# gillesdegottex/percivaltts

Hardware: AMD Instinct MI355X
Metric: acoustic frames/sec per WGAN-GP critic+gen step (higher is better)
Workload: dtype f32

## Files before the change

include/percival_hip.h:

```cpp
#ifndef PERCIVAL_HIP_H
#define PERCIVAL_HIP_H

#include <stddef.h>
#include <stdint.h>

#ifdef __cplusplus
extern "C" {
#endif

#define PTTS_OK            0
#define PTTS_EINVAL       -1
#define PTTS_ELAUNCH      -2
#define PTTS_EWORKSPACE   -3
#define PTTS_EDEVICE      -4

#define PTTS_IN_NONE     0
#define PTTS_IN_LRELU    1
#define PTTS_IN_MASKMUL  2

#define PTTS_PAD_SAME    0
#define PTTS_PAD_CAUSAL  1

#define PTTS_ACT_NONE    0
#define PTTS_ACT_LRELU   1
// ... 126 lines not shown
                                     int Kin, int N, int M, long long lda, long long ldb, int in_mode, float alpha,
                                     void* stream);
int ptts_dense_wgrad_reduce_grouped(const ptts_dense_wgrad_reduce_desc* descs, int n, void* stream);
int ptts_dense_wgrad_bf16x6(const float* A, const float* dY, const float* mask_src, const float* in_scale,
                            const float* in_shift, float* C, float* colsum_b, void* workspace, size_t workspace_bytes,
                            int Kin, int N, int M, long long lda, long long ldb, long long ldc, int in_mode, float alpha,
                            void* stream);
int ptts_dense_bf16x6(const float* A, const void* planes, const float* bias, float* C, int M, int N, int K,
                      long long lda, long long ldc, int in_mode, const float* in_scale, const float* in_shift,
                      const float* mask_src, float alpha, int accumulate, const float* out_mask, void* stream);
int ptts_dense_bf16x6_res(const float* A, const void* planes, const float* bias, float* C, int M, int N, int K,
                          long long lda, long long ldc, int in_mode, const float* in_scale, const float* in_shift,
                          const float* mask_src, float alpha, const float* res, int res_rows, long long ldr,
                          const float* out_mask, void* stream);
int ptts_dense_bf16x6_stats_rows(int M, int N);
int ptts_dense_bf16x6_stats(const float* A, const void* planes, const float* bias, float* C, int M, int N, int K,
                            long long lda, long long ldc, int in_mode, const float* in_scale, const float* in_shift,
                            float alpha, double* stats, int capacity_rows, int* nrows_out, void* stream);
int ptts_dense_bf16x6_bwd_affine(const float* A, const void* planes, float* C, int M, int N, int K, long long lda, long long ldc,
                                 const float* z, const float* scale, const float* shift, float alpha,
                                 double* stats, int capacity_rows, int* nrows_out, void* stream);
int ptts_partial_rows_sum(const double* partials, int nrows, int ncols, double* out, void* stream);
int ptts_dft_mirror(float* Ap, int NB, int B, int Cin, int Kh, void* stream);

int ptts_conv1d_freq_kernel_planes(const float* w, const float* tw, void* planes, int NB, int KW, int Cin, int N, int Kh, void* stream);

int ptts_transpose_batched(const float* src, float* dst, int nb, int rows, int cols, void* stream);
int ptts_conv1d_freq_wgrad_combine(const float* out2, float* dW, int KW, int Cin, int N, int Kh, void* stream);

size_t ptts_conv1d_freq_wgrad_inverse_workspace_bytes(int KW, int Cin, int N);
int ptts_conv1d_freq_wgrad_inverse(const float* Gt, const float* t2, float* dW, void* workspace, size_t workspace_bytes,
                                   int NB, int NBp, int KW, int Cin, int N, int Kh, void* stream);

int ptts_dense_bf16x6_batched(const float* A, long long strideA, const void* planes, long long stride_planes_bytes,
                              const float* bias, float* C, long long strideC, int nbatch, int M, int N, int K,
                              long long lda, long long ldc, int planes_count, void* stream);
int ptts_set_dense_batched_resident(int on);
int ptts_dense_batched_resident_eligible(long long strideA, int M, int N, int K, int planes_count);
int ptts_dense_tn_bf16x6_batched(const float* A, long long strideA, const float* B, long long strideB, float* C, long long strideC,
                                 int nbatch, int M, int Kin, int N, long long lda, long long ldb, long long ldc, int planes_count,
                                 void* stream);

int ptts_split3_frames(const float* x, void* p1, void* p2, void* p3, int B, int T, int C, int pad_left, int pad_right,
                       int Cp, void* stream);
int ptts_split3_weight_t(const float* w, void* p1, void* p2, void* p3, int KW, int C, int N, int Cp, void* stream);
int ptts_conv1d_bf16x6(const void* a1, const void* a2, const void* a3, const void* bt1, const void* bt2, const void* bt3,
                       const float* bias, float* y, int B, int T, int KW, int Cp, int N, void* stream);

int ptts_split3_frames_t(const float* x, void* p1, void* p2, void* p3, int B, int T, int C, int pad_left, int Tp, int Crows,
                         long long Pp, void* stream);
int ptts_conv1d_wgrad_bf16x6(const void* xt1, const void* xt2, const void* xt3, const void* yt1, const void* yt2,
                             const void* yt3, float* dw, int B, int T, int KW, int C, int N, int Crows, long long Pp,
                             void* stream);

int ptts_transpose_frames(const float* x, float* out, int B, int T, int C, int pad_left, int Tp, int Crows, long long Pp,
                          void* stream);
int ptts_conv1d_wgrad_t(const float* xt, const float* yt, float* dw, float* db, int B, int T, int KW, int C, int N, int Crows,
                        long long Pp, void* stream);

size_t ptts_colstats_workspace_bytes(long long rows, int C);
int ptts_colstats(const float* x, long long rows, int C,
                  int in_mode, const float* in_scale, const float* in_shift, const float* mask_src, float alpha,
                  double* sums , void* workspace, size_t workspace_bytes, void* stream);

int ptts_bn_finalize(const double* sums, long long count, const float* gamma, const float* beta,
                     float* moving_mean, float* moving_var, float eps, float momentum,
                     int training, int update_moving, int unbiased_moving, int C,
                     float* scale, float* shift, float* mean , float* rstd , void* stream);

int ptts_bn_batch_stats_supported(long long rows, int C);
// ... 168 lines not shown
```

percivaltts_amd/_hip.py:

```python
import ctypes
import os
import re

import torch

_HERE = os.path.dirname(os.path.abspath(__file__))
LIB_PATH = os.environ.get('PTTS_LIB_PATH') or os.path.join(_HERE, 'lib', 'libpercival_hip.so')
HEADER_PATH = os.environ.get('PTTS_HEADER_PATH') or os.path.join(_HERE, '..', 'include', 'percival_hip.h')


class HipLibraryError(RuntimeError):
    pass


_SCALARS = {'int': ctypes.c_int, 'unsigned': ctypes.c_uint, 'float': ctypes.c_float, 'double': ctypes.c_double,
            'size_t': ctypes.c_size_t, 'long long': ctypes.c_longlong, 'unsigned long long': ctypes.c_ulonglong}
_DECLARATOR = re.compile(r'(.*[\s*])(\w+)\s*(\[\s*\])?', re.S)


def _ctype(spelling, where):
    t = ' '.join(w for w in spelling.replace('*', ' * ').split() if w != 'const')
    if t.endswith('*'):
        return ctypes.c_char_p if t == 'char *' else ctypes.c_void_p
    if t not in _SCALARS:
# ... 23 lines not shown
                raise HipLibraryError('percival_hip.h: cannot read {!r}'.format(' '.join(line.split())))
            fields.extend((n.strip(), ctype) for n in [name] + more)
        return ''

    text = re.sub(r'typedef\s+struct\s+(\w+)\s*\{(.*?)\}\s*\1\s*;', struct, text, flags=re.S)
    for decl in filter(str.strip, text.split(';')):
        m = re.fullmatch(r'\s*(.+?)\b(ptts_\w+)\s*\((.*)\)\s*', decl, flags=re.S)
        if m is None:
            raise HipLibraryError('percival_hip.h: cannot read {!r}'.format(' '.join(decl.split())))
        args = [] if m.group(3).strip() == 'void' else [_declaration(a, decl)[1] for a in m.group(3).split(',')]
        functions[m.group(2)] = (_ctype(m.group(1), decl), args)
    return structs, functions


def read_header(path):
    if not os.path.exists(path):
        raise HipLibraryError('percival_hip.h not found at {}: it lies in include/ beside the package (or set PTTS_HEADER_PATH). '
                              'The binding is read from it.'.format(path))
    with open(path) as f:
        return parse_header(f.read())


_STRUCTS, SIGNATURES = read_header(HEADER_PATH)


def _structure(name, cname):
    return type(name, (ctypes.Structure,), {'_fields_': _STRUCTS[cname], '__doc__': 'struct {} of include/percival_hip.h.'.format(cname)})


WGradDesc = _structure('WGradDesc', 'ptts_wgrad_desc')
DenseWgradReduceDesc = _structure('DenseWgradReduceDesc', 'ptts_dense_wgrad_reduce_desc')
DenseSplitDesc = _structure('DenseSplitDesc', 'ptts_dense_split_desc')
Conv2dReduceDesc = _structure('Conv2dReduceDesc', 'ptts_conv2d_reduce_desc')

_lib = None


def lib():
    global _lib
    if _lib is None:
        if not os.path.exists(LIB_PATH):
            raise HipLibraryError(
                'libpercival_hip.so not found at {}: run `python -c "import __graft_entry__ as g; g.build()"` '
                '(or `make -C percivaltts_amd/csrc`). There is no CPU fallback.'.format(LIB_PATH))
        l = ctypes.CDLL(LIB_PATH)
        for name, (res, args) in SIGNATURES.items():
            fn = getattr(l, name)
            fn.restype = res
            fn.argtypes = args
        if os.environ.get('PTTS_DETERMINISTIC', '0') == '1':
            l.ptts_set_deterministic(1)
        _lib = l
    return _lib


def last_error():
    return lib().ptts_last_error().decode('utf8', 'replace')


class KernelTimer(object):
    active = None

    def __init__(self):
        self.records = []

    def __enter__(self):
# ... 72 lines not shown
```

percivaltts_amd/csrc/dense.hip:

```cpp
#include "common.h"
#include <cstdlib>

namespace ptts {
namespace dns {

typedef __bf16 bf16x8 __attribute__((ext_vector_type(8)));
typedef __bf16 bf16x4 __attribute__((ext_vector_type(4)));
typedef __bf16 bf16x2 __attribute__((ext_vector_type(2)));
typedef float f32x4 __attribute__((ext_vector_type(4)));
typedef float f32x2 __attribute__((ext_vector_type(2)));
typedef unsigned u32x2 __attribute__((ext_vector_type(2)));
typedef unsigned short u16;

constexpr int THREADS = 512;
constexpr int NBLK = 256;
constexpr int BK = 32;

#define DNS_PRODUCTS(X) X(2, 0) X(1, 1) X(0, 2) X(1, 0) X(0, 1) X(0, 0)
#define DNS_PRODUCTS_NPL(NPL, X) do { if (NPL == 3) { X(2, 0) X(1, 1) X(0, 2) X(1, 0) X(0, 1) } X(0, 0) } while (0)

__device__ __forceinline__ unsigned pk_bf16(float a, float b) {
    return __builtin_bit_cast(unsigned, __builtin_convertvector((f32x2){a, b}, bf16x2));
}
__device__ __forceinline__ void split3_pair(float a, float b, unsigned& p1, unsigned& p2, unsigned& p3) {
// ... 509 lines not shown
                for (int e = 0; e < 4; ++e) { row[n + e] = (double)ssum[e]; row[g.N + n + e] = (double)ssq[e]; }
            }
        }
    }
}

template <int MODE, bool AFFINE, int MT, int NPL>
static void dense_launch_kernel(bool xt, dim3 grid, hipStream_t st, const DenseArgs& g) {
    if constexpr (MT < 8) {
        if (xt) { hipLaunchKernelGGL((dense_bf16x6_kernel<MODE, AFFINE, MT, NPL, true>), grid, dim3(THREADS), 0, st, g); return; }
    }
    hipLaunchKernelGGL((dense_bf16x6_kernel<MODE, AFFINE, MT, NPL>), grid, dim3(THREADS), 0, st, g);
}

static int pick_mt(int M, int col_blocks) {
    static int forced = -1;
    if (forced < 0) { const char* e = getenv("PTTS_DENSE_MT"); forced = e ? atoi(e) : 0; }
    if (forced >= 4 && forced <= 8) return forced;
    int best = 8; double best_eff = -1.0;
    for (int mt = 4; mt <= 8; ++mt) {
        const long long blocks = (long long)((M + 16 * mt - 1) / (16 * mt)) * col_blocks;
        const long long rounds = (blocks + 255) / 256;
        const double eff = (double)M * col_blocks / (double)(rounds * 256 * 16 * mt);
        if (eff > best_eff + 1e-9) { best_eff = eff; best = mt; }
    }
    return best;
}

constexpr int RES_M = 128, RES_K = 128;
constexpr int RES_KS = RES_K / BK;
constexpr int RES_PL = RES_M * BK;
template <int NPL> constexpr size_t resident_lds_bytes() { return (size_t)RES_KS * NPL * RES_PL * sizeof(u16); }

template <int NPL, int MT = RES_M / 16, int KSC = 0>
__global__ __launch_bounds__(THREADS) void dense_bf16x6_resident_kernel(DenseArgs g, int slices, int items) {
    extern __shared__ __attribute__((aligned(16))) u16 lds_r[];
    const int tid = threadIdx.x, lane = tid & 63;
    const int wave = __builtin_amdgcn_readfirstlane(tid >> 6);
    const int li = lane & 15, lg = lane >> 4;
    const int KS = KSC ? KSC : g.KS;
    const size_t ps = (size_t)g.NT * KS * 512;
    const int stride = 8 * (int)gridDim.x;
    int item = 8 * (int)blockIdx.x + wave;
    const bool live = item < items;

    constexpr int NQ = RES_M * (RES_K / 4) / THREADS;
    f32x4 va[NQ];
#pragma unroll
    for (int j = 0; j < NQ; ++j) {
        const int q = tid + j * THREADS, row = q >> 5, k4 = 4 * (q & 31);
        const bool ok = row < g.M && k4 < g.K;
        va[j] = *reinterpret_cast<const f32x4*>(g.A + (ok ? (long long)row * g.lda + k4 : 0));
    }

    bf16x8 wf[RES_KS][2][NPL];
    auto load_w = [&](int it, int s) {
        const int z = it / slices, sl = it - z * slices;
        const u16* wp = g.planes + (long long)z * g.bsP + (((size_t)(2 * sl) * KS + s) * 64 + lane) * 8;
#pragma unroll
        for (int j = 0; j < 2; ++j)
#pragma unroll
            for (int p = 0; p < NPL; ++p) wf[s][j][p] = *reinterpret_cast<const bf16x8*>(wp + p * ps + (size_t)j * KS * 512);
    };
#pragma unroll
    for (int s = 0; s < RES_KS; ++s) {
        if (s < KS) load_w(live ? item : items - 1, s);
        __builtin_amdgcn_sched_barrier(0);
    }

    {
#pragma unroll
        for (int j = 0; j < NQ; ++j) {
            const int q = tid + j * THREADS, row = q >> 5, s = (q & 31) >> 3, kq = q & 7;
            u16* d = lds_r + s * NPL * RES_PL + row * BK + ((((kq >> 1) ^ ((row >> 1) & 2))) << 3) + (kq & 1) * 4;
            const f32x4 a = (row < g.M && 4 * (q & 31) < g.K) ? va[j] : f32x4{0.f, 0.f, 0.f, 0.f};
            if (NPL == 3) {
                unsigned a1, a2, a3, b1, b2, b3;
                split3_pair(a[0], a[1], a1, a2, a3);
                split3_pair(a[2], a[3], b1, b2, b3);
                *reinterpret_cast<u32x2*>(d) = (u32x2){a1, b1};
                *reinterpret_cast<u32x2*>(d + RES_PL) = (u32x2){a2, b2};
                *reinterpret_cast<u32x2*>(d + 2 * RES_PL) = (u32x2){a3, b3};
            } else {
                *reinterpret_cast<u32x2*>(d) = (u32x2){pk_bf16(a[0], a[1]), pk_bf16(a[2], a[3])};
            }
        }
    }
    __syncthreads();
    if (!live) return;

    const int boff = li * BK + ((lg ^ ((li >> 1) & 2)) << 3);
    auto run_item = [&](const int it, const bool has_next, const int next) __attribute__((always_inline)) {
        const int z = it / slices, sl = it - z * slices;
        f32x4 bv[2] = {f32x4{0.f, 0.f, 0.f, 0.f}, f32x4{0.f, 0.f, 0.f, 0.f}};
        if (g.bias) {
#pragma unroll
            for (int j = 0; j < 2; ++j)
#pragma unroll
                for (int e = 0; e < 4; ++e) bv[j][e] = g.bias[min(32 * sl + 16 * j + 4 * lg + e, g.N - 1)];
        }
        f32x4 acc[MT][2];
#pragma unroll
        for (int i = 0; i < MT; ++i) { acc[i][0] = f32x4{0.f, 0.f, 0.f, 0.f}; acc[i][1] = f32x4{0.f, 0.f, 0.f, 0.f}; }
#pragma unroll
        for (int s = 0; s < RES_KS; ++s) {
            if (s < KS) {
                const u16* as = lds_r + s * NPL * RES_PL + boff;
#pragma unroll
                for (int i = 0; i < MT; ++i) {
                    bf16x8 bf[NPL];
#pragma unroll
                    for (int p = 0; p < NPL; ++p) bf[p] = *reinterpret_cast<const bf16x8*>(as + p * RES_PL + i * 16 * BK);
#define DNS_MM(PA, PW)                                                                                    \
                    acc[i][0] = __builtin_amdgcn_mfma_f32_16x16x32_bf16(wf[s][0][PW < NPL ? PW : 0], bf[PA < NPL ? PA : 0], acc[i][0], 0, 0, 0);    \
                    acc[i][1] = __builtin_amdgcn_mfma_f32_16x16x32_bf16(wf[s][1][PW < NPL ? PW : 0], bf[PA < NPL ? PA : 0], acc[i][1], 0, 0, 0);
                    DNS_PRODUCTS_NPL(NPL, DNS_MM);
#undef DNS_MM
                }
                if (has_next) load_w(next, s);
                if (KSC) __builtin_amdgcn_sched_barrier(0);
            }
        }
        float* __restrict__ Cz = g.C + (long long)z * g.bsC;
#pragma unroll
        for (int j = 0; j < 2; ++j) {
            const int n = 32 * sl + 16 * j + 4 * lg;
            if (n >= g.N) continue;
            if (g.vec_out && n + 3 < g.N) {
#pragma unroll
                for (int i = 0; i < MT; ++i) {
                    const int m = 16 * i + li;
                    if (m < g.M) *reinterpret_cast<f32x4*>(Cz + (long long)m * g.ldc + n) = acc[i][j] + bv[j];
                }
            } else {
#pragma unroll
                for (int e = 0; e < 4; ++e) {
                    if (n + e >= g.N) continue;
#pragma unroll
                    for (int i = 0; i < MT; ++i) {
                        const int m = 16 * i + li;
                        if (m < g.M) Cz[(long long)m * g.ldc + n + e] = acc[i][j][e] + bv[j][e];
                    }
                }
            }
        }
    };
    int next = item + stride;
    run_item(item, next < items, next);
    while (next < items) {
        item = next;
        next = item + stride;
        run_item(item, next < items, next);
    }
}


typedef short s16x4 __attribute__((ext_vector_type(4)));
typedef s16x4 __attribute__((address_space(3)))* lds_s16x4_ptr;
__device__ __forceinline__ bf16x4 tr_read(const u16* p) {
    return __builtin_bit_cast(bf16x4, __builtin_amdgcn_ds_read_tr16_b64_v4i16((lds_s16x4_ptr)(p)));
}
__device__ __forceinline__ bf16x8 cat8(bf16x4 a, bf16x4 b) { return __builtin_shufflevector(a, b, 0, 1, 2, 3, 4, 5, 6, 7); }

struct WgradArgs {
    const float* A; const float* dY; const float* mask_src; const float* in_scale; const float* in_shift;
    float* partials;
    int Kin, N, M;
    long long lda, ldb;
    float alpha;
    int tiles_n, steps_total, split;
    int tiles_k, part;
};

constexpr int WT = 128;
constexpr int WROW = WT;
constexpr int WPL = 32 * WROW;
constexpr int WPART = WT * WT + WT;
constexpr int WXR = 16;
constexpr int WXPL = 32 * WXR + 4 * 64;
constexpr int WPARTX = WXR * WT;
__host__ __device__ inline bool wgrad_has_rem(int Kin) { return Kin > WT && Kin % WT >= 1 && Kin % WT <= WXR; }
__host__ __device__ inline int wgrad_tiles_k(int Kin) { return wgrad_has_rem(Kin) ? Kin / WT : (Kin + WT - 1) / WT; }
__host__ __device__ inline int wgrad_part(int Kin) { return WPART + (wgrad_has_rem(Kin) ? WPARTX : 0); }

template <int MODE, bool AFFINE, int NPL, bool XR = false>
// ... 612 lines not shown

extern "C" int ptts_conv1d_freq_kernel_planes(const float* w, const float* tw, void* planes, int NB, int KW, int Cin, int N, int Kh,
                                              void* stream) {
    PTTS_REQUIRE(w && tw && planes && NB > 0 && Cin > 0 && N > 0, "conv1d_freq_kernel_planes: bad arguments");
    PTTS_REQUIRE(Kh >= Cin && Kh % 8 == 0, "conv1d_freq_kernel_planes: Kh=%d must be a multiple of 8 and >= Cin=%d", Kh, Cin);
    const int NT = (N + NBLK - 1) / NBLK * (NBLK / 16), KS = (2 * Kh + BK - 1) / BK;
    const long long total = (long long)NT * KS * 64;
    const long long fstride = (long long)(ptts_dense_planes_bytes(N, 2 * Kh) / sizeof(u16));
    const dim3 grid((unsigned)((total + 255) / 256), (unsigned)((NB + WDFT_FCH - 1) / WDFT_FCH));
#define WDFT(KWv) hipLaunchKernelGGL(conv1d_wdft_planes_kernel<KWv>, grid, dim3(256), 0, (hipStream_t)stream, w, tw, (u16*)planes, fstride, NB, Cin, N, Kh, NT, KS)
    switch (KW) {
        case 3: WDFT(3); break;
        case 5: WDFT(5); break;
        case 7: WDFT(7); break;
        case 9: WDFT(9); break;
        case 11: WDFT(11); break;
        case 21: WDFT(21); break;
        default: set_error("conv1d_freq_kernel_planes: KW=%d not instantiated (3, 5, 7, 9, 11, 21)", KW); return PTTS_EINVAL;
    }
#undef WDFT
    return check_launch("conv1d_freq_kernel_planes");
}

static int g_batched_resident = -1;
static int batched_resident_on() {
    if (g_batched_resident < 0) { const char* e = getenv("PTTS_DENSE_BATCHED_RESIDENT"); g_batched_resident = e ? (atoi(e) != 0 ? 1 : 0) : 1; }
    return g_batched_resident;
}
extern "C" int ptts_set_dense_batched_resident(int on) {
    const int prev = batched_resident_on();
    g_batched_resident = on ? 1 : 0;
    return prev;
}
extern "C" int ptts_dense_batched_resident_eligible(long long strideA, int M, int N, int K, int planes_count) {
    return (strideA == 0 && M > 0 && M <= RES_M && N > 0 && K > 0 && K <= RES_K && K % 4 == 0 &&
            (planes_count == 1 || planes_count == 3)) ? 1 : 0;
}

template <int NPL, int MT>
static void resident_set_lds() {
    (void)hipFuncSetAttribute(reinterpret_cast<const void*>(&dense_bf16x6_resident_kernel<NPL, MT, 0>), hipFuncAttributeMaxDynamicSharedMemorySize,
                              (int)resident_lds_bytes<NPL>());
    (void)hipFuncSetAttribute(reinterpret_cast<const void*>(&dense_bf16x6_resident_kernel<NPL, MT, RES_KS>), hipFuncAttributeMaxDynamicSharedMemorySize,
                              (int)resident_lds_bytes<NPL>());
    if constexpr (MT > 1) resident_set_lds<NPL, MT - 1>();
}
static int resident_cus() {
    constexpr int MAXDEV = 64;
    static int cus[MAXDEV];
    int dev = 0;
    if (hipGetDevice(&dev) != hipSuccess || dev < 0 || dev >= MAXDEV) { set_error("dense_bf16x6_batched: no current device"); return 0; }
    if (!cus[dev]) {
        int n = 0;
        if (hipDeviceGetAttribute(&n, hipDeviceAttributeMultiprocessorCount, dev) != hipSuccess || n <= 0) {
            set_error("dense_bf16x6_batched: the device does not tell its compute units"); return 0;
        }
        resident_set_lds<3, RES_M / 16>();
        resident_set_lds<1, RES_M / 16>();
        cus[dev] = n;
    }
    return cus[dev];
}
static int resident_launch(DenseArgs g, int slices, int items, int planes_count, hipStream_t st) {
    const int cus = resident_cus();
    if (!cus) return PTTS_ELAUNCH;
    const int wgs = (items + 7) / 8;
    const dim3 grid((unsigned)(wgs < cus ? wgs : cus));
#define DNS_RK(NPL, MT) do { if (g.KS == RES_KS) hipLaunchKernelGGL((dense_bf16x6_resident_kernel<NPL, MT, RES_KS>), grid, dim3(THREADS), resident_lds_bytes<NPL>(), st, g, slices, items); \
                             else hipLaunchKernelGGL((dense_bf16x6_resident_kernel<NPL, MT, 0>), grid, dim3(THREADS), resident_lds_bytes<NPL>(), st, g, slices, items); } while (0)
#define DNS_R(MT) do { if (planes_count == 1) DNS_RK(1, MT); else DNS_RK(3, MT); } while (0)
    switch ((g.M + 15) / 16) {
        case 1: DNS_R(1); break;
        case 2: DNS_R(2); break;
        case 3: DNS_R(3); break;
        case 4: DNS_R(4); break;
        case 5: DNS_R(5); break;
        case 6: DNS_R(6); break;
        case 7: DNS_R(7); break;
        default: DNS_R(8); break;
    }
#undef DNS_R
#undef DNS_RK
    return check_launch("dense_bf16x6_batched");
}

extern "C" int ptts_dense_bf16x6_batched(const float* A, long long strideA, const void* planes, long long stride_planes_bytes,
                                         const float* bias, float* C, long long strideC, int nbatch, int M, int N, int K,
                                         long long lda, long long ldc, int planes_count, void* stream) {
    PTTS_REQUIRE(A && planes && C && nbatch > 0 && nbatch <= 65535, "dense_bf16x6_batched: bad arguments");
    PTTS_REQUIRE(ptts_dense_bf16x6_supported(M, N, K, lda, ldc), "dense_bf16x6_batched: unsupported shape M=%d N=%d K=%d lda=%lld ldc=%lld", M, N, K, lda, ldc);
    PTTS_REQUIRE(lda >= K && ldc >= N && planes_count >= 1 && planes_count <= 3 && planes_count != 2, "dense_bf16x6_batched: bad leading dims / planes");
    PTTS_REQUIRE(stride_planes_bytes % 16 == 0 && strideA % 4 == 0 && ((uintptr_t)A & 15) == 0, "dense_bf16x6_batched: strides of A / planes must keep 16-byte alignment");
    const bool vec_out = N % 4 == 0 && ldc % 4 == 0 && strideC % 4 == 0 && ((uintptr_t)C & 15) == 0 && (!bias || ((uintptr_t)bias & 15) == 0);
    DenseArgs g;
    g.A = A; g.mask_src = nullptr; g.in_scale = nullptr; g.in_shift = nullptr; g.planes = (const u16*)planes; g.bias = bias;
    g.out_mask = nullptr; g.C = C; g.M = M; g.N = N; g.K = K;
    g.NT = (N + NBLK - 1) / NBLK * (NBLK / 16); g.KS = (K + BK - 1) / BK;
    g.lda = lda; g.ldc = ldc; g.alpha = 0.f; g.out_alpha = 0.f; g.accumulate = 0; g.has_affine = 0; g.vec_out = vec_out;
    g.res = nullptr; g.res_rows = 1; g.ldr = 0;
    g.bsA = strideA; g.bsP = stride_planes_bytes / 2; g.bsC = strideC;
    g.stats = nullptr; g.om_scale = g.om_shift = nullptr;
    const long long items = (long long)nbatch * ((N + 31) / 32);
    if (batched_resident_on() && ptts_dense_batched_resident_eligible(strideA, M, N, K, planes_count) && items <= 0x3fffffffLL) {
        g.vec_out = ldc % 4 == 0 && strideC % 4 == 0 && ((uintptr_t)C & 15) == 0 && (!bias || ((uintptr_t)bias & 15) == 0);
        return resident_launch(g, (N + 31) / 32, (int)items, planes_count, (hipStream_t)stream);
    }
    const int cb = (N + NBLK - 1) / NBLK;
    int mt = 8; double best_eff = -1.0;
    {
        static int forced = -1;
        if (forced < 0) { const char* e = getenv("PTTS_DENSE_BATCHED_MT"); forced = e ? atoi(e) : 0; }
        for (int m = 8; m >= 4; --m) {
            const int tiles = (M + 16 * m - 1) / (16 * m);
            const double eff = (double)M / (double)(tiles * 16 * m);
            if (eff > best_eff + 1e-9) { best_eff = eff; mt = m; }
        }
        if (forced >= 4 && forced <= 8) mt = forced;
    }
    const dim3 grid((unsigned)((M + 16 * mt - 1) / (16 * mt)), (unsigned)cb, (unsigned)nbatch);
    hipStream_t st = (hipStream_t)stream;
    const bool one = planes_count == 1;
#define DNS_B(MT) do { if (one) hipLaunchKernelGGL((dense_bf16x6_kernel<PTTS_IN_NONE, false, MT, 1>), grid, dim3(THREADS), 0, st, g); \
                       else hipLaunchKernelGGL((dense_bf16x6_kernel<PTTS_IN_NONE, false, MT, 3>), grid, dim3(THREADS), 0, st, g); } while (0)
    switch (mt) {
        case 4: DNS_B(4); break;
        case 5: DNS_B(5); break;
        case 6: DNS_B(6); break;
        case 7: DNS_B(7); break;
        default: DNS_B(8); break;
    }
#undef DNS_B
    return check_launch("dense_bf16x6_batched");
}

extern "C" int ptts_dense_tn_bf16x6_batched(const float* A, long long strideA, const float* B, long long strideB, float* C,
                                            long long strideC, int nbatch, int M, int Kin, int N, long long lda, long long ldb,
                                            long long ldc, int planes_count, void* stream) {
    PTTS_REQUIRE(A && B && C && nbatch > 0 && nbatch <= 65535, "dense_tn_bf16x6_batched: bad arguments");
    PTTS_REQUIRE(M > 0 && Kin > 0 && N > 0, "dense_tn_bf16x6_batched: bad shape M=%d Kin=%d N=%d", M, Kin, N);
// ... 132 lines not shown
```

percivaltts_amd/ops.py:

```python
import contextlib
import ctypes
import os

import torch

from . import _hip
from ._hip import call, ptr, stream, f32c, _workspace
from .ops_offline import *

IN_NONE, IN_LRELU, IN_MASKMUL = 0, 1, 2
PAD_SAME, PAD_CAUSAL = 0, 1
ACT_NONE, ACT_LRELU, ACT_SIGMOID, ACT_TANH = 0, 1, 2, 3
ACT_CODES = {None: ACT_NONE, 'linear': ACT_NONE, 'lrelu': ACT_LRELU, 'sigmoid': ACT_SIGMOID, 'tanh': ACT_TANH}


class Lazy(object):
    __slots__ = ('z', 'scale', 'shift', 'lrelu', 'alpha')

    def __init__(self, z, scale=None, shift=None, lrelu=False, alpha=0.3):
        self.z, self.scale, self.shift, self.lrelu, self.alpha = z, scale, shift, lrelu, alpha

    @property
    def shape(self):
        return self.z.shape
# ... 1275 lines not shown
        Pp = _C1Split.plane_len(B, Tp - (KW - 1), KW)
        Crows = (C + 63) // 64 * 64
        key = None if src is None else (src._version, tuple(src.shape), KW, _hip.stream_id())
        if src is not None and cls.src is src and cls.key == key:
            return cls.planes
        xt = torch.empty((Crows, Pp), dtype=torch.float32, device=ap.device)
        call('ptts_transpose_frames', ptr(ap), ptr(xt), B, Tp, C, 0, Tp, Crows, Pp, stream(), tag=(B, Tp, C))
        out = (xt, Crows, Pp)
        if src is not None:
            cls.src, cls.key, cls.planes = src, key, out
        return out

    @classmethod
    def clear(cls):
        cls.src = cls.key = cls.planes = None


def clear_caches():
    _C1Split.clear()
    _C1FFT.clear()
    _C1WgradT.clear()
    _C2M.clear()
    _C2C.clear()
    _DenseSplit.clear()
    _C1Cache.key = _C1Cache.ap = _C1Cache.y = None


class _C1FFT(object):
    default = os.environ.get('PTTS_CONV1D_FFT', '1') == '1'
    enabled = default
    KWS = (3, 5, 7, 9, 11, 21)
    wgrad_enabled = os.environ.get('PTTS_CONV1D_FFT_WGRAD', '1') == '1'
    tn_enabled = os.environ.get('PTTS_CONV1D_FFT_TN', '1') == '1'
    bf16_one_product = os.environ.get('PTTS_CONV1D_FFT_BF16', '1') == '1'
    seg_target = int(os.environ.get('PTTS_CONV1D_FFT_SEG', '100'))
    consts = {}
    x_src = None; x_key = None; x_hat = None
    xw_src = None; xw_key = None; xw_planes = None
    w_hat = {}
    bufs = {}

    @staticmethod
    def eligible(a, w):
        B, T, Cin = a.shape
        KW, _, N = w.shape
        if not (a.is_cuda and B * T >= 4096 and KW >= 3 and KW % 2 == 1 and T % 4 == 0 and N % 4 == 0 and Cin >= 64):
            return False
        return B * (T // _C1FFT.segment(T, KW)) <= 65535

    @classmethod
    def segment(cls, T, KW):
        tgt = cls.seg_target
        if tgt <= 0:
            return T
        best = T
        for S in range(4, T + 1, 4):
            if T % S == 0 and S >= 2 * KW and abs(S - tgt) < abs(best - tgt):
                best = S
        return best

    @classmethod
    def _buf(cls, name, key, nfloats, dev):
        sid = _hip.stream_id()
        k = (name, key, sid)
        t = cls.bufs.get(k)
        if t is None:
# ... 19 lines not shown
        import math
        S = cls.segment(T, KW)
        NS = T // S
        P = (S + KW - 1 + 3) // 4 * 4
        NB = P // 2 + 1
        pl = (KW - 1) // 2
        f = torch.arange(NB, dtype=torch.float64).view(NB, 1)
        i = torch.arange(P, dtype=torch.float64).view(1, P)
        th = 2.0 * math.pi * torch.remainder(f * i, P) / P
        D = torch.stack([torch.cos(th), -torch.sin(th)], dim=1).reshape(2 * NB, P)
        cf = torch.full((NB,), 2.0, dtype=torch.float64); cf[0] = 1.0; cf[P // 2] = 1.0
        R = 2 * NB
        Rp = (R + 3) // 4 * 4
        E = torch.zeros(S, Rp, dtype=torch.float64)
        E[:, 0:R:2] = (torch.cos(th[:, :S]) * cf.view(NB, 1) / P).t()
        E[:, 1:R:2] = (-torch.sin(th[:, :S]) * cf.view(NB, 1) / P).t()
        k = torch.arange(KW, dtype=torch.float64).view(1, KW)
        tk = 2.0 * math.pi * torch.remainder(f * k, P) / P
        Tw = torch.stack([torch.cos(tk), torch.sin(tk)], dim=1).reshape(R, KW)
        NBp = (NB + 3) // 4 * 4
        T2 = torch.zeros(2 * KW, NBp, dtype=torch.float64)
        T2[:KW, :NB] = (torch.cos(tk) * cf.view(NB, 1) / P).t()
        T2[KW:, :NB] = (torch.sin(tk) * cf.view(NB, 1) / P).t()
        TP = (2 * KW + 15) // 16 * 16
        T2f = torch.zeros(NB, TP, dtype=torch.float64)
        T2f[:, :2 * KW] = T2[:, :NB].t()
        to = lambda m: m.to(torch.float32).to(dev).contiguous()
        c = {'S': S, 'NS': NS, 'P': P, 'NB': NB, 'R': R, 'Rp': Rp, 'NBp': NBp, 'TP': TP, 'pl': pl, 'Kh': (Cin + 7) // 8 * 8,
             'D': to(D), 'E': to(E), 'Tw': to(Tw), 'T2': to(T2), 'T2f': to(T2f)}
        cls.consts[key] = c
        return c

    @classmethod
    def x_transform(cls, a, KW):
        B, T, Cin = a.shape
        key = (a._version, tuple(a.shape), KW, _hip.stream_id())
        if cls.x_src is a and cls.x_key == key:
            return cls.x_hat
        c = cls.const(T, KW, Cin, a.device)
        NB, Kh, NS, S, P = c['NB'], c['Kh'], c['NS'], c['S'], c['P']
        Z = B * NS
        Ap = cls._buf('Ap', (B, T, Cin, KW, S), NB * 2 * Z * 2 * Kh, a.device)
        lib = _hip.lib()
        npb = lib.ptts_dense_planes_bytes(Cin, P)
        xpl = cls._scratch('xpl', Z * npb, a.device)
        call('ptts_split3_frame_windows', ptr(a), B, T, Cin, NS, S, -c['pl'], P, P, ptr(xpl), npb, stream(), tag=('x', Z))
        call('ptts_dense_bf16x6_batched', ptr(c['D']), 0, ptr(xpl), npb, None, ptr(Ap), 2 * Kh, Z, c['R'], Cin, P, P, Z * 2 * Kh, 3, stream(),
             tag=('dft', Z, c['R'], Cin, P))
        call('ptts_dft_mirror', ptr(Ap), NB, Z, Cin, Kh, stream())
        cls.x_src, cls.x_key, cls.x_hat = a, key, Ap
        return Ap

    @classmethod
    def kernel(cls, w, T):
        KW, Cin, N = w.shape
        flat = getattr(w, '_ptts_flat', None)
        epoch = None if flat is None else flat.epoch
        sid = _hip.stream_id()
        c = cls.const(T, KW, Cin, w.device)
        NB, Kh = c['NB'], c['Kh']
        geo = (c['S'], NB, Kh)
        ent = cls.w_hat.get((id(w), sid))
        if ent is not None and ent[0] is w and ent[1] == w._version and ent[2] == epoch and flat is not None and ent[5] == geo:
            if cls.frozen_log is not None and id(flat) in cls.frozen:
                cls.frozen_log.append((w, ent[4], T))
            return ent[4]
        lib = _hip.lib()
        npb = lib.ptts_dense_planes_bytes(N, 2 * Kh)
        if ent is not None and ent[0] is w and ent[5] == geo:
            planes = ent[4]
        else:
            planes = torch.empty(NB * npb, dtype=torch.uint8, device=w.device)
        cls._build_kernel_planes(w, c, planes)
        if len(cls.w_hat) >= 8 and (id(w), sid) not in cls.w_hat:
            cls.w_hat = {k: e for k, e in cls.w_hat.items() if id(getattr(e[0], '_ptts_flat', None)) in cls.frozen}
        cls.w_hat[(id(w), sid)] = (w, w._version, epoch, None, planes, geo, T)
# ... 5 lines not shown
        NB, Kh = c['NB'], c['Kh']
        if KW in cls.KWS:
            call('ptts_conv1d_freq_kernel_planes', ptr(w), ptr(c['Tw']), ptr(planes), NB, KW, Cin, N, Kh, stream(), tag=(NB, KW, Cin, N))
        else:
            npb = _hip.lib().ptts_dense_planes_bytes(N, 2 * Kh)
            What = torch.zeros(c['R'] * Kh * N, dtype=torch.float32, device=w.device)
            gemm_raw(c['Tw'], w.view(KW, Cin * N), What, c['R'], Cin * N, KW, lda=KW, ldb=Cin * N, ldc=Kh * N)
            call('ptts_split3_dense_weight_strided', ptr(What), 2 * Kh * N, ptr(planes), npb, NB, N, 2 * Kh, N, 0, stream(), tag=('w', NB))

    frozen = set()
    frozen_log = None

    @classmethod
    def refresh_planes(cls, items):
        for w, planes, T in items:
            KW, Cin, N = w.shape
            cls._build_kernel_planes(w, cls.const(T, KW, Cin, w.device), planes)
        return len(items)

    @classmethod
    def forward(cls, a, w, b, y):
        B, T, Cin = a.shape
        KW, _, N = w.shape
        c = cls.const(T, KW, Cin, a.device)
        NB, Kh, NS, S = c['NB'], c['Kh'], c['NS'], c['S']
        Z = B * NS
        lib = _hip.lib()
        Ap = cls.x_transform(a, KW)
        wpl = cls.kernel(w, T)
        npw = lib.ptts_dense_planes_bytes(N, 2 * Kh)
        Yh = cls._scratch('Yh', NB * 2 * Z * N * 4, a.device)
        call('ptts_dense_bf16x6_batched', ptr(Ap), 2 * Z * 2 * Kh, ptr(wpl), npw, None, ptr(Yh), 2 * Z * N, NB, 2 * Z, N, 2 * Kh,
             2 * Kh, N, 1 if _Flags.bf16_products else 3, stream(), tag=('freq', NB, 2 * Z, N, 2 * Kh))
        npy = lib.ptts_dense_planes_bytes(N, c['R'])
        ypl = cls._scratch('ypl', Z * npy, a.device)
        call('ptts_split3_dense_weight_strided', ptr(Yh), N, ptr(ypl), npy, Z, Z * N, c['R'], N, 0, stream(), tag=('y', Z))
        call('ptts_dense_bf16x6_batched', ptr(c['E']), 0, ptr(ypl), npy, ptr(b), ptr(y), S * N, Z, S, N, c['Rp'], c['Rp'], N, 3, stream(),
             tag=('idft', Z, S, N, c['Rp']))

    @classmethod
    def has_x(cls, a, KW):
        return a is not None and cls.x_src is a and cls.x_key == (a._version, tuple(a.shape), KW, _hip.stream_id())

    @classmethod
    def wgrad(cls, a, dy, KW):
        B, T, Cin = a.shape
        N = dy.shape[-1]
        c = cls.const(T, KW, Cin, a.device)
        NB, Kh, NS, S, P = c['NB'], c['Kh'], c['NS'], c['S'], c['P']
        Z = B * NS
        lib = _hip.lib()
        dev = a.device
        Ap = cls.x_hat
        npd = lib.ptts_dense_planes_bytes(N, P)
        dpl = cls._scratch('dpl', Z * npd, dev)
        call('ptts_split3_frame_windows', ptr(dy), B, T, N, NS, S, 0, P, S, ptr(dpl), npd, stream(), tag=('dy', Z))
        DYh = cls._scratch('DYh', NB * 2 * Z * N * 4, dev)
        call('ptts_dense_bf16x6_batched', ptr(c['D']), 0, ptr(dpl), npd, None, ptr(DYh), N, Z, c['R'], N, P, P, Z * N, 3, stream(),
             tag=('dft_dy', Z, c['R'], N, P))
        Gt = cls._scratch('Gt', NB * N * 2 * Kh * 4, dev)
        if cls.tn_enabled and not _Flags.bf16_products:
            call('ptts_dense_tn_bf16x6_batched', ptr(DYh), 2 * Z * N, ptr(Ap), 2 * Z * 2 * Kh, ptr(Gt), N * 2 * Kh, NB, 2 * Z, N, 2 * Kh, N, 2 * Kh,
                 2 * Kh, 3, stream(), tag=('corr', NB, N, 2 * Kh, 2 * Z))
        else:
            npx = lib.ptts_dense_planes_bytes(2 * Kh, 2 * Z)
            if cls.xw_src is not a or cls.xw_key != cls.x_key or cls.xw_planes is None:
                xw = cls._scratch('xw', NB * npx, dev)
                call('ptts_split3_dense_weight_strided', ptr(Ap), 2 * Z * 2 * Kh, ptr(xw), npx, NB, 2 * Kh, 2 * Z, 2 * Kh, 0, stream(), tag=('xw', NB))
                cls.xw_src, cls.xw_key, cls.xw_planes = a, cls.x_key, xw
            DYt = cls._scratch('DYt', NB * N * 2 * Z * 4, dev)
            call('ptts_transpose_batched', ptr(DYh), ptr(DYt), NB, 2 * Z, N, stream())
            call('ptts_dense_bf16x6_batched', ptr(DYt), N * 2 * Z, ptr(cls.xw_planes), npx, None, ptr(Gt), N * 2 * Kh, NB, N, 2 * Kh, 2 * Z,
                 2 * Z, 2 * Kh, 1 if _Flags.bf16_products else 3, stream(), tag=('corr', NB, N, 2 * Kh, 2 * Z))
        dw = torch.empty((KW, Cin, N), dtype=torch.float32, device=dev)
        if KW in cls.KWS:
            ws = _workspace(lib.ptts_conv1d_freq_wgrad_inverse_workspace_bytes(KW, Cin, N), dev)
            call('ptts_conv1d_freq_wgrad_inverse', ptr(Gt), ptr(c['T2f']), ptr(dw), ptr(ws), ws.numel(), NB, c['TP'], KW, Cin, N, Kh, stream(),
                 tag=(NB, KW, Cin, N))
        else:
            out2 = torch.empty(2 * KW * N * 2 * Kh, dtype=torch.float32, device=dev)
            gemm_raw(c['T2'], Gt[:NB * N * 2 * Kh * 4].view(torch.float32), out2, 2 * KW, N * 2 * Kh, NB, lda=c['NBp'], ldb=N * 2 * Kh, ldc=N * 2 * Kh)
            call('ptts_conv1d_freq_wgrad_combine', ptr(out2), ptr(dw), KW, Cin, N, Kh, stream())
        return dw

    @classmethod
    def clear(cls):
        cls.x_src = cls.x_key = cls.x_hat = None
        cls.xw_src = cls.xw_key = cls.xw_planes = None
        cls.w_hat = {k: (e if id(getattr(e[0], '_ptts_flat', None)) in cls.frozen else (e[0], None, None, e[3], e[4], e[5]) + tuple(e[6:]))
                     for k, e in cls.w_hat.items()}


def conv1d_fft(on):
    _C1FFT.enabled = _C1FFT.default if on is None else bool(on)
    _C1FFT.clear()


def conv1d_split(on):
    _C1Split.enabled = _C1Split.default if on is None else bool(on)
    _C1Split.clear()


class Conv1dFn(torch.autograd.Function):
    @staticmethod
    def forward(ctx, a, w, b, pre=None):
        f32c(a, 'conv1d.a'); f32c(w, 'conv1d.w')
        B, T, Cin = a.shape
        KW, Ci2, N = w.shape
        assert Ci2 == Cin
        pl = (KW - 1) // 2
        if pre is not None:
            saved, padded, y = pre
        else:
            y = torch.empty((B, T, N), dtype=torch.float32, device=a.device)
            if _C1FFT.enabled and _C1Split.enabled and (not _Flags.bf16_products or _C1FFT.bf16_one_product) and _C1FFT.eligible(a, w):
                _C1FFT.forward(a, w, b, y)
                saved, padded = a, False
            elif _C1Split.enabled and not _Flags.deterministic and _C1Split.eligible(a, w):
                xp, Cp = _C1Split.frames(a, pl, KW - 1 - pl)
                wp = _C1Split.kernel(w)
                call('ptts_conv1d_bf16x6', ptr(xp[0]), ptr(xp[1]), ptr(xp[2]), ptr(wp[0]), ptr(wp[1]), ptr(wp[2]), ptr(b), ptr(y),
                     B, T, KW, Cp, N, stream(), tag=(B, T, KW, Cp, N))
                saved, padded = a, False
            else:
                saved, padded = _pad_time(a, pl, KW - 1 - pl), True
                gemm_raw(saved, w, y, B * T, N, KW * Cin, lda=Cin, rows_per_seg=T, seg_stride=(T + KW - 1) * Cin, bias=b)
            if _C1Cache.capture:
# ... 662 lines not shown
```

Measured before the change: 4.846 million.

## Fuse fp32-to-bf16 split of right operand into resident dense kernel for FFT conv

```diff
diff --git a/include/percival_hip.h b/include/percival_hip.h
--- a/include/percival_hip.h
+++ b/include/percival_hip.h
@@ -182,10 +182,18 @@
 int ptts_conv1d_freq_wgrad_inverse(const float* Gt, const float* t2, float* dW, void* workspace, size_t workspace_bytes,
                                    int NB, int NBp, int KW, int Cin, int N, int Kh, void* stream);
 
+#define PTTS_PLANES_ROWS 0x100
+typedef struct ptts_dense_rows_desc {
+    const float* B;
+    long long strideB, ldb;
+    int windows, nB, T, NS, S, row_off;
+    int kvalid, mirror_cols;
+} ptts_dense_rows_desc;
 int ptts_dense_bf16x6_batched(const float* A, long long strideA, const void* planes, long long stride_planes_bytes,
                               const float* bias, float* C, long long strideC, int nbatch, int M, int N, int K,
                               long long lda, long long ldc, int planes_count, void* stream);
 int ptts_set_dense_batched_resident(int on);
+int ptts_dense_batched_resident_enabled(void);
 int ptts_dense_batched_resident_eligible(long long strideA, int M, int N, int K, int planes_count);
 int ptts_dense_tn_bf16x6_batched(const float* A, long long strideA, const float* B, long long strideB, float* C, long long strideC,
                                  int nbatch, int M, int Kin, int N, long long lda, long long ldb, long long ldc, int planes_count,
diff --git a/percivaltts_amd/_hip.py b/percivaltts_amd/_hip.py
--- a/percivaltts_amd/_hip.py
+++ b/percivaltts_amd/_hip.py
@@ -79,6 +79,18 @@
 DenseWgradReduceDesc = _structure('DenseWgradReduceDesc', 'ptts_dense_wgrad_reduce_desc')
 DenseSplitDesc = _structure('DenseSplitDesc', 'ptts_dense_split_desc')
 Conv2dReduceDesc = _structure('Conv2dReduceDesc', 'ptts_conv2d_reduce_desc')
+DenseRowsDesc = _structure('DenseRowsDesc', 'ptts_dense_rows_desc')
+
+
+def _define(name):
+    with open(HEADER_PATH) as f:
+        m = re.search(r'^[ \t]*#[ \t]*define[ \t]+{}[ \t]+(\w+)'.format(name), f.read(), flags=re.M)
+    if m is None:
+        raise HipLibraryError('percival_hip.h: no #define {}'.format(name))
+    return int(m.group(1), 0)
+
+
+PLANES_ROWS = _define('PTTS_PLANES_ROWS')
 
 _lib = None
 
diff --git a/percivaltts_amd/csrc/dense.hip b/percivaltts_amd/csrc/dense.hip
--- a/percivaltts_amd/csrc/dense.hip
+++ b/percivaltts_amd/csrc/dense.hip
@@ -565,9 +565,17 @@
 constexpr int RES_PL = RES_M * BK;
 template <int NPL> constexpr size_t resident_lds_bytes() { return (size_t)RES_KS * NPL * RES_PL * sizeof(u16); }
 
-template <int NPL, int MT = RES_M / 16, int KSC = 0>
-__global__ __launch_bounds__(THREADS) void dense_bf16x6_resident_kernel(DenseArgs g, int slices, int items) {
+struct RowsArgs {
+    const float* B; long long strideB;
+    int ldb, windows, T, NS, S, row_off, kvalid, mirror;
+};
+template <bool ROWS> struct RowsItemT { unsigned base[2], len[2], t0; };
+template <> struct RowsItemT<false> {};
+
+template <int NPL, int MT = RES_M / 16, int KSC = 0, bool ROWS = false>
+__global__ __launch_bounds__(THREADS) void dense_bf16x6_resident_kernel(DenseArgs g, int slices, int items, RowsArgs r) {
     extern __shared__ __attribute__((aligned(16))) u16 lds_r[];
+    using RowsItem = RowsItemT<ROWS>;
     const int tid = threadIdx.x, lane = tid & 63;
     const int wave = __builtin_amdgcn_readfirstlane(tid >> 6);
     const int li = lane & 15, lg = lane >> 4;
@@ -595,9 +603,50 @@
 #pragma unroll
             for (int p = 0; p < NPL; ++p) wf[s][j][p] = *reinterpret_cast<const bf16x8*>(wp + p * ps + (size_t)j * KS * 512);
     };
+    float wr[ROWS ? RES_KS : 1][2][8];
+    auto rows_item = [&](int it) {
+        RowsItem q;
+        if constexpr (ROWS) {
+            const int z = it / slices, sl = it - z * slices;
+            long long zoff; int rlo = 0, rhi = r.kvalid;
+            if (r.windows) {
+                const int b = z / r.NS, sg = z - b * r.NS;
+                const int r0 = r.row_off + sg * r.S;
+                zoff = ((long long)b * r.T + r0) * r.ldb;
+                rlo = r0 < 0 ? -r0 : 0;
+                rhi = min(r.kvalid, r.T - r0);
+            } else {
+                zoff = (long long)z * r.strideB;
+            }
+            const unsigned len = (unsigned)max(rhi - rlo, 0);
+            q.t0 = (unsigned)(8 * lg - rlo);
+#pragma unroll
+            for (int j = 0; j < 2; ++j) {
+                const int n = 32 * sl + 16 * j + li;
+                q.len[j] = n < g.N ? len : 0u;
+                q.base[j] = 4u * ((unsigned)zoff + (unsigned)(8 * lg) * (unsigned)r.ldb + (unsigned)n);
+            }
+        }
+        return q;
+    };
+    auto load_r = [&](const RowsItem& q, int s) {
+        if constexpr (ROWS) {
+            const unsigned ldb4 = 4u * (unsigned)r.ldb;
+            unsigned a[2] = {q.base[0] + 32u * s * ldb4, q.base[1] + 32u * s * ldb4};
+#pragma unroll
+            for (int e = 0; e < 8; ++e)
+#pragma unroll
+                for (int j = 0; j < 2; ++j) {
+                    const unsigned c = 32 * s + e;
+                    wr[ROWS ? s : 0][j][e] = *reinterpret_cast<const float*>(reinterpret_cast<const char*>(r.B) + (q.t0 + c < q.len[j] ? a[j] : 0u));
+                    a[j] += ldb4;
+                }
+        }
+    };
+    RowsItem qcur = rows_item(live ? item : items - 1);
 #pragma unroll
     for (int s = 0; s < RES_KS; ++s) {
-        if (s < KS) load_w(live ? item : items - 1, s);
+        if (s < KS) { if constexpr (ROWS) load_r(qcur, s); else load_w(live ? item : items - 1, s); }
         __builtin_amdgcn_sched_barrier(0);
     }
 
@@ -623,7 +672,7 @@
     if (!live) return;
 
     const int boff = li * BK + ((lg ^ ((li >> 1) & 2)) << 3);
-    auto run_item = [&](const int it, const bool has_next, const int next) __attribute__((always_inline)) {
+    auto run_item = [&](const int it, const bool has_next, const int next, const RowsItem& qc, const RowsItem& qn) __attribute__((always_inline)) {
         const int z = it / slices, sl = it - z * slices;
         f32x4 bv[2] = {f32x4{0.f, 0.f, 0.f, 0.f}, f32x4{0.f, 0.f, 0.f, 0.f}};
         if (g.bias) {
@@ -639,18 +688,37 @@
         for (int s = 0; s < RES_KS; ++s) {
             if (s < KS) {
                 const u16* as = lds_r + s * NPL * RES_PL + boff;
+                bf16x8 ws[2][NPL];
+                if constexpr (ROWS) {
+#pragma unroll
+                    for (int j = 0; j < 2; ++j) {
+                        unsigned q[3][4];
+#pragma unroll
+                        for (int h = 0; h < 4; ++h) {
+                            const unsigned c = 32 * s + 2 * h;
+                            const float v0 = qc.t0 + c < qc.len[j] ? wr[ROWS ? s : 0][j][2 * h] : 0.f;
+                            const float v1 = qc.t0 + c + 1 < qc.len[j] ? wr[ROWS ? s : 0][j][2 * h + 1] : 0.f;
+                            if (NPL == 3) split3_pair(v0, v1, q[0][h], q[1][h], q[2][h]);
+                            else q[0][h] = pk_bf16(v0, v1);
+                        }
+#pragma unroll
+                        for (int p = 0; p < NPL; ++p) ws[j][p] = __builtin_bit_cast(bf16x8, make_uint4(q[p][0], q[p][1], q[p][2], q[p][3]));
+                    }
+                }
 #pragma unroll
                 for (int i = 0; i < MT; ++i) {
                     bf16x8 bf[NPL];
 #pragma unroll
                     for (int p = 0; p < NPL; ++p) bf[p] = *reinterpret_cast<const bf16x8*>(as + p * RES_PL + i * 16 * BK);
+#define DNS_WF(J, PW) (ROWS ? ws[J][PW < NPL ? PW : 0] : wf[s][J][PW < NPL ? PW : 0])
 #define DNS_MM(PA, PW)                                                                                    \
-                    acc[i][0] = __builtin_amdgcn_mfma_f32_16x16x32_bf16(wf[s][0][PW < NPL ? PW : 0], bf[PA < NPL ? PA : 0], acc[i][0], 0, 0, 0);    \
-                    acc[i][1] = __builtin_amdgcn_mfma_f32_16x16x32_bf16(wf[s][1][PW < NPL ? PW : 0], bf[PA < NPL ? PA : 0], acc[i][1], 0, 0, 0);
+                    acc[i][0] = __builtin_amdgcn_mfma_f32_16x16x32_bf16(DNS_WF(0, PW), bf[PA < NPL ? PA : 0], acc[i][0], 0, 0, 0);    \
+                    acc[i][1] = __builtin_amdgcn_mfma_f32_16x16x32_bf16(DNS_WF(1, PW), bf[PA < NPL ? PA : 0], acc[i][1], 0, 0, 0);
                     DNS_PRODUCTS_NPL(NPL, DNS_MM);
 #undef DNS_MM
+#undef DNS_WF
                 }
-                if (has_next) load_w(next, s);
+                if (has_next) { if constexpr (ROWS) load_r(qn, s); else load_w(next, s); }
                 if (KSC) __builtin_amdgcn_sched_barrier(0);
             }
         }
@@ -663,7 +731,11 @@
 #pragma unroll
                 for (int i = 0; i < MT; ++i) {
                     const int m = 16 * i + li;
-                    if (m < g.M) *reinterpret_cast<f32x4*>(Cz + (long long)m * g.ldc + n) = acc[i][j] + bv[j];
+                    if (m < g.M) {
+                        const f32x4 v = acc[i][j] + bv[j];
+                        *reinterpret_cast<f32x4*>(Cz + (long long)m * g.ldc + n) = v;
+                        if (ROWS && r.mirror > 0) *reinterpret_cast<f32x4*>(Cz + (long long)(m ^ 1) * g.ldc + r.mirror + n) = (li & 1) ? -v : v;
+                    }
                 }
             } else {
 #pragma unroll
@@ -672,18 +744,26 @@
 #pragma unroll
                     for (int i = 0; i < MT; ++i) {
                         const int m = 16 * i + li;
-                        if (m < g.M) Cz[(long long)m * g.ldc + n + e] = acc[i][j][e] + bv[j][e];
+                        if (m < g.M) {
+                            const float v = acc[i][j][e] + bv[j][e];
+                            Cz[(long long)m * g.ldc + n + e] = v;
+                            if (ROWS && r.mirror > 0) Cz[(long long)(m ^ 1) * g.ldc + r.mirror + n + e] = (li & 1) ? -v : v;
+                        }
                     }
                 }
             }
         }
     };
     int next = item + stride;
-    run_item(item, next < items, next);
+    RowsItem qnext = qcur;
+    if (ROWS && next < items) qnext = rows_item(next);
+    run_item(item, next < items, next, qcur, qnext);
     while (next < items) {
         item = next;
         next = item + stride;
-        run_item(item, next < items, next);
+        qcur = qnext;
+        if (ROWS && next < items) qnext = rows_item(next);
+        run_item(item, next < items, next, qcur, qnext);
     }
 }
 
@@ -1362,18 +1442,19 @@
     g_batched_resident = on ? 1 : 0;
     return prev;
 }
+extern "C" int ptts_dense_batched_resident_enabled(void) { return batched_resident_on(); }
 extern "C" int ptts_dense_batched_resident_eligible(long long strideA, int M, int N, int K, int planes_count) {
     return (strideA == 0 && M > 0 && M <= RES_M && N > 0 && K > 0 && K <= RES_K && K % 4 == 0 &&
             (planes_count == 1 || planes_count == 3)) ? 1 : 0;
 }
 
-template <int NPL, int MT>
+template <int NPL, int MT, bool ROWS>
 static void resident_set_lds() {
-    (void)hipFuncSetAttribute(reinterpret_cast<const void*>(&dense_bf16x6_resident_kernel<NPL, MT, 0>), hipFuncAttributeMaxDynamicSharedMemorySize,
+    (void)hipFuncSetAttribute(reinterpret_cast<const void*>(&dense_bf16x6_resident_kernel<NPL, MT, 0, ROWS>), hipFuncAttributeMaxDynamicSharedMemorySize,
                               (int)resident_lds_bytes<NPL>());
-    (void)hipFuncSetAttribute(reinterpret_cast<const void*>(&dense_bf16x6_resident_kernel<NPL, MT, RES_KS>), hipFuncAttributeMaxDynamicSharedMemorySize,
+    (void)hipFuncSetAttribute(reinterpret_cast<const void*>(&dense_bf16x6_resident_kernel<NPL, MT, RES_KS, ROWS>), hipFuncAttributeMaxDynamicSharedMemorySize,
                               (int)resident_lds_bytes<NPL>());
-    if constexpr (MT > 1) resident_set_lds<NPL, MT - 1>();
+    if constexpr (MT > 1) resident_set_lds<NPL, MT - 1, ROWS>();
 }
 static int resident_cus() {
     constexpr int MAXDEV = 64;
@@ -1385,19 +1466,23 @@
         if (hipDeviceGetAttribute(&n, hipDeviceAttributeMultiprocessorCount, dev) != hipSuccess || n <= 0) {
             set_error("dense_bf16x6_batched: the device does not tell its compute units"); return 0;
         }
-        resident_set_lds<3, RES_M / 16>();
-        resident_set_lds<1, RES_M / 16>();
+        resident_set_lds<3, RES_M / 16, false>();
+        resident_set_lds<1, RES_M / 16, false>();
+        resident_set_lds<3, RES_M / 16, true>();
+        resident_set_lds<1, RES_M / 16, true>();
         cus[dev] = n;
     }
     return cus[dev];
 }
-static int resident_launch(DenseArgs g, int slices, int items, int planes_count, hipStream_t st) {
+static int resident_launch(DenseArgs g, int slices, int items, int planes_count, const RowsArgs* rows, hipStream_t st) {
     const int cus = resident_cus();
     if (!cus) return PTTS_ELAUNCH;
     const int wgs = (items + 7) / 8;
     const dim3 grid((unsigned)(wgs < cus ? wgs : cus));
-#define DNS_RK(NPL, MT) do { if (g.KS == RES_KS) hipLaunchKernelGGL((dense_bf16x6_resident_kernel<NPL, MT, RES_KS>), grid, dim3(THREADS), resident_lds_bytes<NPL>(), st, g, slices, items); \
-                             else hipLaunchKernelGGL((dense_bf16x6_resident_kernel<NPL, MT, 0>), grid, dim3(THREADS), resident_lds_bytes<NPL>(), st, g, slices, items); } while (0)
+    const RowsArgs r = rows ? *rows : RowsArgs{};
+#define DNS_RKR(NPL, MT, KSC) do { if (rows) hipLaunchKernelGGL((dense_bf16x6_resident_kernel<NPL, MT, KSC, true>), grid, dim3(THREADS), resident_lds_bytes<NPL>(), st, g, slices, items, r); \
+                                   else hipLaunchKernelGGL((dense_bf16x6_resident_kernel<NPL, MT, KSC, false>), grid, dim3(THREADS), resident_lds_bytes<NPL>(), st, g, slices, items, r); } while (0)
+#define DNS_RK(NPL, MT) do { if (g.KS == RES_KS) DNS_RKR(NPL, MT, RES_KS); else DNS_RKR(NPL, MT, 0); } while (0)
 #define DNS_R(MT) do { if (planes_count == 1) DNS_RK(1, MT); else DNS_RK(3, MT); } while (0)
     switch ((g.M + 15) / 16) {
         case 1: DNS_R(1); break;
@@ -1411,16 +1496,41 @@
     }
 #undef DNS_R
 #undef DNS_RK
+#undef DNS_RKR
     return check_launch("dense_bf16x6_batched");
 }
 
 extern "C" int ptts_dense_bf16x6_batched(const float* A, long long strideA, const void* planes, long long stride_planes_bytes,
                                          const float* bias, float* C, long long strideC, int nbatch, int M, int N, int K,
                                          long long lda, long long ldc, int planes_count, void* stream) {
+    const bool rows = (planes_count & PTTS_PLANES_ROWS) != 0;
+    planes_count &= ~PTTS_PLANES_ROWS;
     PTTS_REQUIRE(A && planes && C && nbatch > 0 && nbatch <= 65535, "dense_bf16x6_batched: bad arguments");
     PTTS_REQUIRE(ptts_dense_bf16x6_supported(M, N, K, lda, ldc), "dense_bf16x6_batched: unsupported shape M=%d N=%d K=%d lda=%lld ldc=%lld", M, N, K, lda, ldc);
     PTTS_REQUIRE(lda >= K && ldc >= N && planes_count >= 1 && planes_count <= 3 && planes_count != 2, "dense_bf16x6_batched: bad leading dims / planes");
-    PTTS_REQUIRE(stride_planes_bytes % 16 == 0 && strideA % 4 == 0 && ((uintptr_t)A & 15) == 0, "dense_bf16x6_batched: strides of A / planes must keep 16-byte alignment");
+    PTTS_REQUIRE((rows || stride_planes_bytes % 16 == 0) && strideA % 4 == 0 && ((uintptr_t)A & 15) == 0, "dense_bf16x6_batched: strides of A / planes must keep 16-byte alignment");
+    RowsArgs ra = {};
+    if (rows) {
+        const ptts_dense_rows_desc& d = *(const ptts_dense_rows_desc*)planes;
+        PTTS_REQUIRE(batched_resident_on() && ptts_dense_batched_resident_eligible(strideA, M, N, K, planes_count),
+                     "dense_bf16x6_batched: the fp32-rows form of the right operand exists on the resident-left kernel only (strideA == 0, M <= %d, K <= %d, "
+                     "the switch on): strideA=%lld M=%d K=%d", RES_M, RES_K, strideA, M, K);
+        PTTS_REQUIRE(d.B && d.ldb >= N && d.kvalid > 0 && d.kvalid <= K, "dense_bf16x6_batched: rows form: bad source, ldb=%lld or kvalid=%d", d.ldb, d.kvalid);
+        long long span;
+        if (d.windows) {
+            PTTS_REQUIRE(d.nB > 0 && d.T > 0 && d.NS > 0 && d.S > 0 && (long long)d.nB * d.NS == nbatch && d.row_off > -(1 << 24) && d.row_off < (1 << 24),
+                         "dense_bf16x6_batched: rows form: bad windows nB=%d T=%d NS=%d S=%d row_off=%d for %d members", d.nB, d.T, d.NS, d.S, d.row_off, nbatch);
+            span = ((long long)d.nB * d.T - 1) * d.ldb + N;
+        } else {
+            PTTS_REQUIRE(d.strideB >= 0, "dense_bf16x6_batched: rows form: negative strideB");
+            span = (long long)(nbatch - 1) * d.strideB + (long long)(d.kvalid - 1) * d.ldb + N;
+        }
+        PTTS_REQUIRE(span <= (1LL << 30), "dense_bf16x6_batched: rows form: the source spans more than 2^30 floats");
+        PTTS_REQUIRE(d.mirror_cols >= 0 && (d.mirror_cols == 0 || (d.mirror_cols % 4 == 0 && d.mirror_cols >= N && (long long)d.mirror_cols + N <= ldc && M % 2 == 0)),
+                     "dense_bf16x6_batched: rows form: mirror_cols=%d needs a multiple of 4, N <= mirror_cols, mirror_cols + N <= ldc and an even M", d.mirror_cols);
+        ra.B = d.B; ra.strideB = d.strideB; ra.ldb = (int)d.ldb; ra.windows = d.windows ? 1 : 0;
+        ra.T = d.T; ra.NS = d.NS; ra.S = d.S; ra.row_off = d.row_off; ra.kvalid = d.kvalid; ra.mirror = d.mirror_cols;
+    }
     const bool vec_out = N % 4 == 0 && ldc % 4 == 0 && strideC % 4 == 0 && ((uintptr_t)C & 15) == 0 && (!bias || ((uintptr_t)bias & 15) == 0);
     DenseArgs g;
     g.A = A; g.mask_src = nullptr; g.in_scale = nullptr; g.in_shift = nullptr; g.planes = (const u16*)planes; g.bias = bias;
@@ -1433,8 +1543,10 @@
     const long long items = (long long)nbatch * ((N + 31) / 32);
     if (batched_resident_on() && ptts_dense_batched_resident_eligible(strideA, M, N, K, planes_count) && items <= 0x3fffffffLL) {
         g.vec_out = ldc % 4 == 0 && strideC % 4 == 0 && ((uintptr_t)C & 15) == 0 && (!bias || ((uintptr_t)bias & 15) == 0);
-        return resident_launch(g, (N + 31) / 32, (int)items, planes_count, (hipStream_t)stream);
-    }
+        if (rows) g.planes = nullptr;
+        return resident_launch(g, (N + 31) / 32, (int)items, planes_count, rows ? &ra : nullptr, (hipStream_t)stream);
+    }
+    PTTS_REQUIRE(!rows, "dense_bf16x6_batched: rows form: too many work items");
     const int cb = (N + NBLK - 1) / NBLK;
     int mt = 8; double best_eff = -1.0;
     {
diff --git a/percivaltts_amd/ops.py b/percivaltts_amd/ops.py
--- a/percivaltts_amd/ops.py
+++ b/percivaltts_amd/ops.py
@@ -1331,6 +1331,8 @@
     KWS = (3, 5, 7, 9, 11, 21)
     wgrad_enabled = os.environ.get('PTTS_CONV1D_FFT_WGRAD', '1') == '1'
     tn_enabled = os.environ.get('PTTS_CONV1D_FFT_TN', '1') == '1'
+    rows_default = int(os.environ.get('PTTS_CONV1D_FFT_ROWS', '3'))
+    rows_sites = rows_default
     bf16_one_product = os.environ.get('PTTS_CONV1D_FFT_BF16', '1') == '1'
     seg_target = int(os.environ.get('PTTS_CONV1D_FFT_SEG', '100'))
     consts = {}
@@ -1416,6 +1418,13 @@
         return c
 
     @classmethod
+    def rows_enabled(cls, site, M, N, K, span):
+        if not (cls.rows_sites & site) or span > (1 << 30):
+            return False
+        lib = _hip.lib()
+        return bool(lib.ptts_dense_batched_resident_enabled() and lib.ptts_dense_batched_resident_eligible(0, M, N, K, 3))
+
+    @classmethod
     def x_transform(cls, a, KW):
         B, T, Cin = a.shape
         key = (a._version, tuple(a.shape), KW, _hip.stream_id())
@@ -1426,6 +1435,12 @@
         Z = B * NS
         Ap = cls._buf('Ap', (B, T, Cin, KW, S), NB * 2 * Z * 2 * Kh, a.device)
         lib = _hip.lib()
+        if cls.rows_enabled(1, c['R'], Cin, P, B * T * Cin):
+            d = _hip.DenseRowsDesc(B=a.data_ptr(), strideB=0, ldb=Cin, windows=1, nB=B, T=T, NS=NS, S=S, row_off=-c['pl'], kvalid=P, mirror_cols=Kh)
+            call('ptts_dense_bf16x6_batched', ptr(c['D']), 0, ctypes.byref(d), 0, None, ptr(Ap), 2 * Kh, Z, c['R'], Cin, P, P, Z * 2 * Kh,
+                 3 | _hip.PLANES_ROWS, stream(), tag=('dft', Z, c['R'], Cin, P))
+            cls.x_src, cls.x_key, cls.x_hat = a, key, Ap
+            return Ap
         npb = lib.ptts_dense_planes_bytes(Cin, P)
         xpl = cls._scratch('xpl', Z * npb, a.device)
         call('ptts_split3_frame_windows', ptr(a), B, T, Cin, NS, S, -c['pl'], P, P, ptr(xpl), npb, stream(), tag=('x', Z))
@@ -1497,6 +1512,11 @@
         Yh = cls._scratch('Yh', NB * 2 * Z * N * 4, a.device)
         call('ptts_dense_bf16x6_batched', ptr(Ap), 2 * Z * 2 * Kh, ptr(wpl), npw, None, ptr(Yh), 2 * Z * N, NB, 2 * Z, N, 2 * Kh,
              2 * Kh, N, 1 if _Flags.bf16_products else 3, stream(), tag=('freq', NB, 2 * Z, N, 2 * Kh))
+        if cls.rows_enabled(2, S, N, c['Rp'], c['R'] * Z * N):
+            d = _hip.DenseRowsDesc(B=Yh.data_ptr(), strideB=N, ldb=Z * N, windows=0, nB=0, T=0, NS=0, S=0, row_off=0, kvalid=c['R'], mirror_cols=0)
+            call('ptts_dense_bf16x6_batched', ptr(c['E']), 0, ctypes.byref(d), 0, ptr(b), ptr(y), S * N, Z, S, N, c['Rp'], c['Rp'], N,
+                 3 | _hip.PLANES_ROWS, stream(), tag=('idft', Z, S, N, c['Rp']))
+            return
         npy = lib.ptts_dense_planes_bytes(N, c['R'])
         ypl = cls._scratch('ypl', Z * npy, a.device)
         call('ptts_split3_dense_weight_strided', ptr(Yh), N, ptr(ypl), npy, Z, Z * N, c['R'], N, 0, stream(), tag=('y', Z))
@@ -1558,6 +1578,11 @@
 
 def conv1d_fft(on):
     _C1FFT.enabled = _C1FFT.default if on is None else bool(on)
+    _C1FFT.clear()
+
+
+def conv1d_fft_rows(on):
+    _C1FFT.rows_sites = _C1FFT.rows_default if on is None else (3 if on is True else int(on))
     _C1FFT.clear()
 
 
```

Result: faster. 4.947 million (median of 6 runs) (+2.1%).
